# horizon-research/Fov-3DGS

Hardware: AMD Instinct MI355X
Metric: frames/sec at 1080p foveated (bicycle-scale) (higher is better)
Workload: dtype f32; 1 GPU; S-6M bicycle-scale cloud, 4-layer foveated render (fov_pcheck_obb), the reference's 9 fixed gazes (0.25 i, 0.25 j) in turn, one camera per GPU; gaussians=6000000, width=1920, height=1080, sh_degree=3, model_layout=the reference's tensor interface (render(packed=None)), overlap_successive_frames=True, parallelism=views1

## Files before the change

fov-3dgs_amd/csrc/api.hip:

```cpp
#include "common.h"
#include <mutex>
#include <cstdarg>
#include <cstdio>
#include <cstring>
#include <cstdlib>
#include <new>

namespace fr {

static thread_local char g_err[512] = "";

void set_error(const char *fmt, ...)
{
	va_list ap;
	va_start(ap, fmt);
	vsnprintf(g_err, sizeof(g_err), fmt, ap);
	va_end(ap);
}

int check_launch(const char *what, hipStream_t stream, bool debug)
{
	hipError_t e = hipGetLastError();
	static const bool trace = getenv("FR_TRACE") != nullptr;
	if (trace) { fprintf(stderr, "[fovraster] launched %s\n", what); fflush(stderr); }
// ... 189 lines not shown
	c.a = a; c.stream = stream;
	if (a->P == 0)
	{
		FR_HIP(hipMemsetAsync(a->out_color, 0, sizeof(float) * 3 * (size_t)a->W * a->H, stream));
		f->empty = true;
		*out = f; guard.f = nullptr;
		return FR_OK;
	}
	auto mark = [&](int i) { if (a->stage_events && a->stage_events[i]) (void)hipEventRecord((hipEvent_t)a->stage_events[i], stream); };
	c.gx = (a->W + FR_TILE - 1) / FR_TILE; c.gy = (a->H + FR_TILE - 1) / FR_TILE; c.T = c.gx * c.gy;
	c.focal_y = a->H / (2.0f * a->tanfovy);
	c.focal_x = a->W / (2.0f * a->tanfovx);

	char *gptr = a->geometry_resize(a->resize_user[0], carve_geom(a->variant, (size_t)a->P, nullptr).bytes);
	char *iptr = a->image_resize(a->resize_user[2], carve_image(a->variant, a->W, a->H, nullptr).bytes);
	if (!gptr || !iptr) { set_error("geometry/image resize callback returned null"); return FR_ERR_ALLOC; }
	c.geom = carve_geom(a->variant, (size_t)a->P, gptr);
	c.img = carve_image(a->variant, a->W, a->H, iptr);

	c.fov_split = a->variant == FR_VARIANT_FOV_PCHECK_OBB ? 1 : 0;
	f->ax = (!a->debug && !a->no_helper_streams) ? aux_stream(stream) : nullptr;
	hipStream_t fill_stream = stream;
	const bool stats = has_stats(a->variant) && !a->no_stats;
	if (f->ax && (c.fov_split || stats))
	{
		if (hipEventRecord(f->ax->fork, stream) != hipSuccess || hipStreamWaitEvent(f->ax->s2, f->ax->fork, 0) != hipSuccess) { (void)hipGetLastError(); f->ax = nullptr; }
		else fill_stream = f->ax->s2;
	}
	auto fills_done = [&]() { if (fill_stream != stream && hipEventRecord(f->ax->join2, f->ax->s2) == hipSuccess) f->aux_pending = true; };
	if (c.fov_split)
	{
		const hipError_t e = hipMemsetAsync(a->out_color, 0, sizeof(float) * 3 * (size_t)a->W * a->H, fill_stream);
		fills_done();
		if (e != hipSuccess) { set_error("hipMemsetAsync(out_color): %s", hipGetErrorString(e)); return FR_ERR_HIP; }
	}
	if (stats)
	{
		const hipError_t e1 = hipMemsetAsync(a->gaussians_count, 0, sizeof(int32_t) * (size_t)a->P, fill_stream);
		const hipError_t e2 = hipMemsetAsync(a->contributions, 0, sizeof(float) * (size_t)a->P, fill_stream);
		fills_done();
		if (e1 != hipSuccess || e2 != hipSuccess) { set_error("hipMemsetAsync(statistics): %s", hipGetErrorString(e1 != hipSuccess ? e1 : e2)); return FR_ERR_HIP; }
	}
	FR_HIP(hipMemsetAsync(c.img.tile_count, 0, (size_t)((char *)(c.img.lv_bbox + 5 * FR_LV_BBOX_STRIDE) - (char *)c.img.tile_count), stream));
	if (!is_fov(a->variant))
		FR_HIP(hipMemsetAsync(c.geom.slab_ctr, 0, FR_SLAB_CTR_WORDS * sizeof(uint32_t), stream));
	if (a->list_consumed) FR_HIP(hipMemsetAsync(a->list_consumed, 0, sizeof(uint32_t) * (size_t)c.T, stream));
	if (a->blend_pairs) FR_HIP(hipMemsetAsync(a->blend_pairs, 0, sizeof(uint32_t) * (size_t)c.T, stream));
	static thread_local uint32_t frame_seq = 0;
	if (++frame_seq == 0) frame_seq = 1;
	c.totals_seq = frame_seq;
	mark(FR_STAGE_TILE_LEVELS);
	if (is_fov(a->variant)) { rc = launch_tile_levels(c); if (rc) return rc; }
	mark(FR_STAGE_PROJECT);
	rc = launch_project(c); if (rc) return rc;
	int cur_dev = 0;
	(void)hipGetDevice(&cur_dev);
	f->pin = a->debug ? nullptr : take_pinned(cur_dev);
	c.totals_host_dev = f->pin ? f->pin->dev : nullptr;
	c.scan_fused = 0;
	mark(FR_STAGE_BIN);
	f->scan_enqueued = true;
	rc = launch_bin(c); if (rc) return rc;
	mark(FR_STAGE_TILE_SCAN);
	if (!c.scan_fused) { rc = launch_tile_scan(c); if (rc) return rc; }
	*out = f; guard.f = nullptr;
	return FR_OK;
}

// ... 43 lines not shown
	a->num_rendered = (int32_t)totals[0];
	a->max_tile_instances = (int32_t)totals[1];
	a->num_candidates = (int32_t)candidates;
	c.heavy4 = (int)totals[2]; c.heavy2 = (int)totals[3];
	c.n_items = (int)totals[5]; c.heavy8 = (int)totals[6];
	const int64_t want = (int64_t)totals[0] + (int64_t)totals[0] / 4 + 65536;
	if (!same_kind) { gs.variant = a->variant; gs.P = a->P; gs.W = a->W; gs.H = a->H; gs.capacity = 0; }
	if (want > gs.capacity) gs.capacity = want;

	const bool fits_early = early_bin && (int64_t)totals[0] <= early_cap;
	const int64_t capacity = fits_early ? early_cap : (int64_t)totals[0];
	char *bptr = fits_early ? early_bin : a->binning_resize(a->resize_user[1], carve_bin(capacity, nullptr, c.T).bytes);
	if (!bptr) { set_error("binning resize callback returned null"); return FR_ERR_ALLOC; }
	c.bin = carve_bin(capacity, bptr, c.T);
	c.capacity = capacity;
	c.items_cap = (int64_t)(c.fov_split ? 4 : 2) * c.T;
	int rc = FR_OK;
	mark(FR_STAGE_EMIT);
	if (a->num_rendered > 0) { rc = launch_emit(c); if (rc) return rc; }
	mark(FR_STAGE_TILE_SORT);
	if (a->num_rendered > 0) { rc = launch_tile_sort(c); if (rc) return rc; }
	mark(FR_STAGE_RENDER);
	f->join_aux();
	rc = launch_render(c);
	mark(FR_NUM_STAGES);
	return rc;
}

int fr_forward_abandon(fr_frame *f)
{
	if (!f) { set_error("null frame"); return FR_ERR_INVALID; }
	delete f;
	return FR_OK;
}

int fr_forward(fr_forward_args *a)
{
	fr_frame *f = nullptr;
	const int rc = fr_forward_begin(a, &f);
	if (rc) return rc;
	return fr_forward_finish(f);
}

int fr_pack_geom(int32_t P, const float *means3D, const float *scales, const float *rotations, const float *opacities,
	int32_t levels, const float *highest_levels, float *packed_geom, void *stream)
{
// ... 106 lines not shown
```

fov-3dgs_amd/csrc/common.h:

```cpp
#pragma once
#include <hip/hip_runtime.h>
#include <stdint.h>
#include <stddef.h>
#include "../../include/fovraster.h"

#define FR_TILE 16
#define FR_TILE_PIX 256
#define FR_FOV_LEVELS 4
#define FR_SORT_LDS_MAX 8192
#ifndef FR_BIN_THREADS
#define FR_BIN_THREADS 768
#endif
#define FR_BIN_BLOCKS 512
#define FR_PROJ_MAX_WAVES 8192
#define FR_CROW_PAD (64 * FR_PROJ_MAX_WAVES)
#define FR_LDS_HIST_MAX_TILES 16384
#define FR_ITEM_NONE 0xffffffffu
#define FR_LDS_HIST16_MAX_TILES 34816
#define FR_HIST16_MAX_SLABS (65535 / FR_BIN_THREADS)
#define FR_BIG_TNUM 64
#define FR_GIANT_TNUM 1024
#define FR_GIANT_MAX 64
#define FR_SORT_SPLIT_MIN 16384
#define FR_SORT_CHUNK_TARGET 960
#define FR_SORT_FINE_BUCKETS 2048
#define FR_SORT_MAX_CHUNKS(D) ((size_t)(D) / FR_SORT_CHUNK_TARGET + (size_t)(D) / FR_SORT_SPLIT_MIN + 16)
#define FR_LV_BBOX_STRIDE 32
#define FR_SLAB_CTR_WORDS 32

namespace fr {

#define FR_VARIANT_SUM_NOSTATS 100
__host__ __device__ inline bool has_stats(int v) { return v == FR_VARIANT_PCHECK_OBB_SUM || v == FR_VARIANT_PCHECK_OBB_MAX || v == FR_VARIANT_PCHECK_OBB_LWMC; }
__host__ __device__ inline bool has_backward(int v) { return v == FR_VARIANT_ORIGINAL || has_stats(v); }
__host__ __device__ constexpr inline bool is_fov(int v) { return v == FR_VARIANT_FOV_PCHECK_OBB || v == FR_VARIANT_NAIVE_FOV_PCHECK_OBB || v == FR_VARIANT_MMFR_PCHECK_OBB; }

__host__ __device__ inline size_t align_up(size_t x, size_t a = 256) { return (x + a - 1) / a * a; }

struct GeomWS {
	float4 *rec;
	float *cov3D;
	float4 *acc;
	float4 *wrec;
	float4 *lvl;
	uint32_t *lrange;
	uint32_t *slab_ctr;
	uint32_t *vis_list;
	uint32_t *vis_seg;
	uint32_t *proj_counts;
	uint32_t *wbase;
// ... 20 lines not shown
	if (variant == FR_VARIANT_FOV_PCHECK_OBB) { g.lvl = (float4 *)(base + off); off = align_up(off + P * FR_FOV_LEVELS * sizeof(float4)); }
	g.lrange = (uint32_t *)(base + off); off = align_up(off + P * sizeof(uint32_t));
	g.slab_ctr = (uint32_t *)(base + off); off = align_up(off + FR_SLAB_CTR_WORDS * sizeof(uint32_t));
	g.vis_list = (uint32_t *)(base + off); off = align_up(off + P * sizeof(uint32_t));
	g.vis_seg = (uint32_t *)(base + off); off = align_up(off + (P + FR_CROW_PAD) * sizeof(uint32_t));
	g.proj_counts = (uint32_t *)(base + off); off = align_up(off + FR_PROJ_MAX_WAVES * sizeof(uint32_t));
	g.wbase = (uint32_t *)(base + off); off = align_up(off + (FR_PROJ_MAX_WAVES + 1) * sizeof(uint32_t));
	g.crow = nullptr;
	if (is_fov(variant)) { g.crow = (float4 *)(base + off); off = align_up(off + (P + FR_CROW_PAD) * 3 * sizeof(float4)); }
	g.rtab = (uint2 *)(base + off); off = align_up(off + (size_t)FR_BIN_BLOCKS * FR_MAX_REGIONS * sizeof(uint2));
	g.wlist = (uint32_t *)(base + off); off = align_up(off + wlist_cap(P) * sizeof(uint32_t));
	g.rtotal = (uint32_t *)(base + off); off = align_up(off + FR_MAX_REGIONS * sizeof(uint32_t));
	g.rchunk = (uint32_t *)(base + off); off = align_up(off + (FR_MAX_REGIONS + 1) * sizeof(uint32_t));
	g.bytes = off + 256;
	return g;
}

struct ImageWS {
	float *final_T;
	uint32_t *n_contrib;
	uint2 *ranges;
	uint32_t *tile_count;
	uint32_t *lv_bbox;
	uint32_t *totals;
	uint32_t *render_items;
	uint32_t *tile_order;
	float *tile_lv;
	uint32_t *hist;
	size_t bytes;
};
__host__ __device__ inline int bin_blocks(int P)
{
	const int slabs = (P + FR_BIN_THREADS - 1) / FR_BIN_THREADS;
	return slabs < FR_BIN_BLOCKS ? (slabs > 0 ? slabs : 1) : FR_BIN_BLOCKS;
}
__host__ __device__ inline ImageWS carve_image(int variant, int W, int H, char *base)
{
	ImageWS s; size_t off = 0;
	const size_t N = (size_t)W * H;
	const size_t T = (size_t)((W + FR_TILE - 1) / FR_TILE) * ((H + FR_TILE - 1) / FR_TILE);
	s.final_T = (float *)(base + off); off = align_up(off + N * sizeof(float));
	s.n_contrib = (uint32_t *)(base + off); off = align_up(off + N * sizeof(uint32_t));
	s.ranges = (uint2 *)(base + off); off = align_up(off + T * sizeof(uint2));
	s.tile_count = (uint32_t *)(base + off); off = align_up(off + T * sizeof(uint32_t));
	s.lv_bbox = (uint32_t *)(base + off); off = align_up(off + 5 * FR_LV_BBOX_STRIDE * sizeof(uint32_t));
	s.totals = (uint32_t *)(base + off); off = align_up(off + 16 * sizeof(uint32_t));
	s.render_items = (uint32_t *)(base + off); off = align_up(off + 4 * T * sizeof(uint32_t));
	s.tile_order = (uint32_t *)(base + off); off = align_up(off + T * sizeof(uint32_t));
	s.tile_lv = nullptr;
	if (is_fov(variant)) { s.tile_lv = (float *)(base + off); off = align_up(off + 5 * T * sizeof(float)); }
	s.hist = nullptr;
	if (T <= FR_LDS_HIST16_MAX_TILES) { s.hist = (uint32_t *)(base + off); off = align_up(off + (size_t)FR_BIN_BLOCKS * T * sizeof(uint32_t)); }
	s.bytes = off + 256;
	return s;
}

struct BinWS {
	uint32_t *point_list;
	uint64_t *entries;
	uint64_t *entries2;
	uint2 *chunks;
	uint32_t *round_flags;
	size_t bytes;
};
__host__ __device__ inline size_t round_flag_words(int64_t D, int64_t T) { return (size_t)((D / 256 + T + 64) / 32 + 1); }
__host__ __device__ inline BinWS carve_bin(int64_t D, char *base, int64_t T = 1 << 20)
{
	BinWS b; size_t off = 0;
	b.point_list = (uint32_t *)(base + off); off = align_up(off + (size_t)D * sizeof(uint32_t));
	b.entries = (uint64_t *)(base + off); off = align_up(off + (size_t)D * sizeof(uint64_t));
	b.entries2 = (uint64_t *)(base + off); off = align_up(off + (size_t)D * sizeof(uint64_t));
	b.chunks = (uint2 *)(base + off); off = align_up(off + FR_SORT_MAX_CHUNKS(D) * sizeof(uint2));
	b.round_flags = (uint32_t *)(base + off); off = align_up(off + round_flag_words(D, T) * sizeof(uint32_t));
// ... 244 lines not shown
```

fov-3dgs_amd/csrc/preprocess.hip:

```cpp
#include "common.h"
#include "tile_scan.h"
#include <cstdlib>

namespace fr {

struct M3 { float c[3][3]; };
__device__ __forceinline__ M3 m3_cols(float a0, float a1, float a2, float b0, float b1, float b2, float c0, float c1, float c2)
{
	M3 m; m.c[0][0] = a0; m.c[0][1] = a1; m.c[0][2] = a2; m.c[1][0] = b0; m.c[1][1] = b1; m.c[1][2] = b2;
	m.c[2][0] = c0; m.c[2][1] = c1; m.c[2][2] = c2; return m;
}
__device__ __forceinline__ M3 m3_mul(const M3 &a, const M3 &b)
{
	M3 r;
#pragma unroll
	for (int col = 0; col < 3; col++)
#pragma unroll
		for (int row = 0; row < 3; row++)
			r.c[col][row] = a.c[0][row] * b.c[col][0] + a.c[1][row] * b.c[col][1] + a.c[2][row] * b.c[col][2];
	return r;
}
__device__ __forceinline__ M3 m3_t(const M3 &a)
{
	M3 r;
// ... 19 lines not shown
	const float nx = px / W, ny = py / H;
	float tdir[3], gdir[3], cdir[3];
	ncd2dir(nx, ny, riw, rih, tdir);
	ncd2dir(gaze_x, gaze_y, riw, rih, gdir);
	ncd2dir(0.5f, 0.5f, riw, rih, cdir);
	const float ecc = acosf(gdir[0] * tdir[0] + gdir[1] * tdir[1] + gdir[2] * tdir[2]);
	const float ecc_c = acosf(tdir[0] * cdir[0] + tdir[1] * cdir[1] + tdir[2] * cdir[2]);
	const float pool = alpha * ecc * ecc;
	const float amin = (float)((double)ecc_c - (double)pool * 0.5);
	const float amax = (float)((double)ecc_c + (double)pool * 0.5);
	const float ax = (float)(((double)nx - 0.5) * (double)riw), ay = (float)(((double)ny - 0.5) * (double)rih);
	const float dist = sqrtf(ax * ax + ay * ay + rvd * rvd);
	const float major = (tanf(amax) - tanf(amin)) * rvd;
	const float minor = 2.0f * dist * tanf(pool * 0.5f);
	const float area = (float)(3.14159265358979323846 * (double)major * (double)minor * (double)0.25f);
	const float r2p = W / riw;
	const float ps = sqrtf(area) * r2p;
	float level;
	if (ps <= 1) level = 0; else level = (sqrtf(ps) - 1) / step;
	if ((double)level > ((double)(float)FR_FOV_LEVELS - 0.1)) level = (float)((double)(float)FR_FOV_LEVELS - 0.1);
	return level;
}

#define FR_LV_PATCH 14
__global__ void __launch_bounds__(256) k_tile_levels(int T, int gx, int gy, int W, int H, float gaze_x, float gaze_y, float alpha, float *out,
	uint32_t *lv_bbox, uint32_t *slab_ctr, float mmfr_level)
{
	if (blockIdx.x == 0)
		for (int i = threadIdx.x; i < FR_SLAB_CTR_WORDS; i += 256) slab_ctr[i] = 0;
	__shared__ float s_lv[16][16];
	const int pxn = (gx + FR_LV_PATCH - 1) / FR_LV_PATCH;
	const int bx = (int)blockIdx.x % pxn, by = (int)blockIdx.x / pxn;
	const int lx = threadIdx.x & 15, ly = threadIdx.x >> 4;
	const int tx = bx * FR_LV_PATCH + lx - 1, ty = by * FR_LV_PATCH + ly - 1;
	const bool in_grid = tx >= 0 && tx < gx && ty >= 0 && ty < gy;
	const bool live = in_grid && lx >= 1 && lx <= FR_LV_PATCH && ly >= 1 && ly <= FR_LV_PATCH;
	const int idx = ty * gx + tx;
	s_lv[ly][lx] = in_grid ? tile_level(tx, ty, W, H, gaze_x, gaze_y, alpha) : -1.0f;
	__syncthreads();
	const float lf = s_lv[ly][lx];
	const int xl = max(lx - 1, 0), xr = min(lx + 1, 15), yd = max(ly - 1, 0), yu = min(ly + 1, 15);
	const float right = s_lv[ly][xr], left = s_lv[ly][xl], up = s_lv[yu][lx], down = s_lv[yd][lx];
	float gxv = 0, gyv = 0;
	if (right != -1 && left != -1) gxv = (right - left) / 2.0f;
	else if (right != -1) gxv = right - lf;
	else if (left != -1) gxv = lf - left;
	if (up != -1 && down != -1) gyv = (up - down) / 2.0f;
	else if (up != -1) gyv = up - lf;
	else if (down != -1) gyv = lf - down;
	const float max_delta = (float)(0.5 * (double)(fabsf(gxv) + fabsf(gyv)));
	const bool mmfr = mmfr_level >= 0.0f;
	float tmin = lf - max_delta;
	if (mmfr && tmin < 0.0f) tmin = 0.0f;
	const float tmin_i = (float)f2i(tmin);
	const bool blending = ((tmin - tmin_i) > 0.5f) && (tmin_i < (float)(FR_FOV_LEVELS - 1));
	const float real_tmin = tmin;
	if (mmfr) tmin = (real_tmin > mmfr_level - 0.5f && real_tmin < mmfr_level + 1.0f) ? 0.0f : 5.0f;
	if (live)
	{
		out[idx] = mmfr ? real_tmin : lf;
		out[T + idx] = tmin;
		out[2 * T + idx] = gxv;
		out[3 * T + idx] = gyv;
		out[4 * T + idx] = blending ? 1.0f : 0.0f;
	}
	__shared__ uint32_t s_bb[(FR_FOV_LEVELS + 1) * 4];
	if (threadIdx.x < (FR_FOV_LEVELS + 1) * 4) s_bb[threadIdx.x] = 0;
	__syncthreads();
	for (int k = 0; k <= FR_FOV_LEVELS; k++)
	{
		const bool in = live && tmin < (float)k;
		uint32_t v[4] = { in ? (uint32_t)(gx - tx) : 0u, in ? (uint32_t)(gy - ty) : 0u, in ? (uint32_t)(tx + 1) : 0u, in ? (uint32_t)(ty + 1) : 0u };
#pragma unroll
		for (int c = 0; c < 4; c++)
		{
#pragma unroll
			for (int off = 32; off > 0; off >>= 1) v[c] = max(v[c], (uint32_t)__shfl_xor((int)v[c], off));
			if ((threadIdx.x & 63) == 0 && v[c] != 0) atomicMax(&s_bb[4 * k + c], v[c]);
		}
	}
	__syncthreads();
	if (threadIdx.x < (FR_FOV_LEVELS + 1) * 4 && s_bb[threadIdx.x] != 0)
		atomicMax(&lv_bbox[(threadIdx.x >> 2) * FR_LV_BBOX_STRIDE + (threadIdx.x & 3)], s_bb[threadIdx.x]);
}

typedef float f4u __attribute__((ext_vector_type(4), aligned(4)));
struct ShRows { f4u v[12]; };
template <bool REST>
__device__ __forceinline__ void sh_fetch(const float *__restrict__ sh, ShRows &r)
{
#pragma unroll
	for (int q = 0; q < 11; q++) r.v[q] = *(const f4u *)(sh + 4 * q);
	if (REST) r.v[11] = (f4u){ sh[44], 0.0f, 0.0f, 0.0f };
	else r.v[11] = *(const f4u *)(sh + 44);
}
__device__ __forceinline__ void sh_basis(float dx, float dy, float dz, float basis[16])
{
	const float len = sqrtf(dx * dx + dy * dy + dz * dz);
	const float x = dx / len, y = dy / len, z = dz / len;
	const float xx = x * x, yy = y * y, zz = z * z;
	const float xy = x * y, yz = y * z, xz = x * z;
	const float b[16] = {
		FR_SH_C0, -(FR_SH_C1 * y), FR_SH_C1 * z, -(FR_SH_C1 * x),
		FR_SH_C2_0 * xy, FR_SH_C2_1 * yz, FR_SH_C2_2 * (2.0f * zz - xx - yy), FR_SH_C2_3 * xz, FR_SH_C2_4 * (xx - yy),
		FR_SH_C3_0 * y * (3.0f * xx - yy), FR_SH_C3_1 * xy * z, FR_SH_C3_2 * y * (4.0f * zz - xx - yy),
		FR_SH_C3_3 * z * (2.0f * zz - 3.0f * xx - 3.0f * yy), FR_SH_C3_4 * x * (4.0f * zz - xx - yy),
// ... 62 lines not shown
	}
#pragma unroll
	for (int ch = 0; ch < 3; ch++) out[ch] = acc[ch] + 0.5f;
}

typedef float nt_f4 __attribute__((ext_vector_type(4)));
__device__ __forceinline__ float4 nt_load4(const float *p)
{
	const nt_f4 v = __builtin_nontemporal_load((const nt_f4 *)p);
	return make_float4(v.x, v.y, v.z, v.w);
}
struct RawGaussian { float p[3], sc[3]; float4 q; float hl; };

#define FR_ER_CHUNK 512
struct PreArgs {
	int P, D, M, W, H, gx, gy;
	float tanfovx, tanfovy, focal_x, focal_y, scale_modifier;
	const float *means3D, *scales, *rotations, *opacities, *shs, *cov3D_precomp, *colors_precomp;
	const float *shs_rest;
	const float *viewmatrix, *projmatrix, *campos;
	const float *shs_dcs, *highest_levels;
	const float *packed_geom, *packed_colour, *packed_cull;
	const float *tile_lv;
	const uint32_t *lv_bbox;
	int lds_tiles;
	int T;
	int *radii;
	GeomWS geom;
	uint32_t *tile_count;
	uint32_t *hist;
	int write_cov3D;
	int raw;
	int prefiltered;
	int proj_waves, proj_cpw;
	int wbase_lds;
	int fuse_scan;
	TileScanArgs ts;
	int regions, region_rx;
	int wcap;
};

struct Proj {
	bool alive;
	float pix_x, pix_y, depth, conic_a, conic_b, conic_c;
	float cov0, cov1, lambda1, lambda2;
	int radius, x0, y0, x1, y1;
	uint32_t tnum;
// ... 212 lines not shown
{
	if (b <= a) return 0ull;
	const unsigned long long hi = b >= 64 ? ~0ull : ((1ull << b) - 1ull);
	return hi & ~((1ull << a) - 1ull);
}

#ifndef FR_PROJ_THREADS
#define FR_PROJ_THREADS 1024
#endif
#ifndef FR_PROJ_DEPTH
#define FR_PROJ_DEPTH 3
#endif
#ifndef FR_PROJ_DEPTH_PACKED
#define FR_PROJ_DEPTH_PACKED 4
#endif
__host__ __device__ inline int proj_chunks_per_wave(int P, int nwaves) { const int nchunks = (P + 63) / 64; return (nchunks + nwaves - 1) / nwaves; }
template <int VARIANT, bool PACKED = false>
__global__ void __launch_bounds__(FR_PROJ_THREADS) k_project(const PreArgs a)
{
	constexpr int DEPTH = PACKED ? FR_PROJ_DEPTH_PACKED : FR_PROJ_DEPTH;
	constexpr bool FOV = VARIANT == FR_VARIANT_FOV_PCHECK_OBB;
	const int lane = threadIdx.x & 63;
	__shared__ uint4 s_lvb[5];
	if (FOV && threadIdx.x < 5) s_lvb[threadIdx.x] = *(const uint4 *)(a.lv_bbox + threadIdx.x * FR_LV_BBOX_STRIDE);
	if (FOV) __syncthreads();
	constexpr bool ROWS = !PACKED && FOV;
	const int nwaves = (int)gridDim.x * (FR_PROJ_THREADS / 64);
	const int nchunks = (a.P + 63) / 64;
	const int wave_gid = (int)blockIdx.x * (FR_PROJ_THREADS / 64) + (int)(threadIdx.x >> 6);
	const int cpw = proj_chunks_per_wave(a.P, nwaves);
	const int c0 = wave_gid * cpw, c1 = min(nchunks, c0 + cpw);
	const uint32_t row_base = (uint32_t)wave_gid * (uint32_t)cpw * 64u;
	uint32_t nrow = 0;
	const bool have_sr = a.cov3D_precomp == nullptr;
	const float wn2 = view_norm2_bound(a.viewmatrix);
	float vm[16], pm[16];
#pragma unroll
	for (int i = 0; i < 16; i++)
	{
		vm[i] = __builtin_bit_cast(float, __builtin_amdgcn_readfirstlane(__builtin_bit_cast(int, a.viewmatrix[i])));
		pm[i] = __builtin_bit_cast(float, __builtin_amdgcn_readfirstlane(__builtin_bit_cast(int, a.projmatrix[i])));
	}
	const float *sc_src = have_sr ? a.scales : a.cov3D_precomp;
	const float *q_src = have_sr ? a.rotations : a.cov3D_precomp;
	bool odd_level = false;
	auto fetch = [&](const int chunk) __attribute__((always_inline))
	{
		const size_t i = (size_t)min(chunk * 64 + lane, a.P - 1);
// ... 762 lines not shown
				if (t == 0) a.geom.rchunk[a.regions] = tot;
			}
		}
	}
}
#undef BUMP_TILE
#undef TILE_FILTER

struct EmitArgs {
	int P, gx, gy, T;
	const int *radii;
	GeomWS geom;
	const float *highest_levels;
	const float *tile_lv;
	const uint32_t *lv_bbox;
	int lds_tiles;
	const uint2 *ranges;
	uint32_t *cursor;
	uint64_t *entries;
	const uint32_t *hist;
	const uint32_t *totals;
	uint32_t capacity;
	uint32_t items_cap;
};
#ifndef FR_EMIT_THREADS
#define FR_EMIT_THREADS FR_BIN_THREADS
#endif
#ifdef FR_EMIT_NOSTORE
#define FR_EMIT_ST(slot, v) do { if ((slot) == 0xffffffffu) a.entries[0] = (v); } while (0)
#elif defined(FR_EMIT_COALESCED)
#define FR_EMIT_ST(slot, v) do { (void)(slot); a.entries[(size_t)blockIdx.x * 20000 + (threadIdx.x & ~63u) * 26u + ((uint32_t)tm_seq++ * 64u + lane) % 1600u] = (v); } while (0)
#else
#define FR_EMIT_ST(slot, v) a.entries[(slot)] = (v)
#endif
#define NEXT_SLOT(ti) (LDSH == 2 ? a.ranges[(ti)].x + pre_row[(ti)] + ((atomicAdd(&lds_cur[(ti) >> 1], 1u << (16 * ((ti) & 1))) >> (16 * ((ti) & 1))) & 0xffffu) \
	: LDSH ? atomicAdd(&lds_cur[(ti)], 1u) : a.ranges[(ti)].x + atomicAdd(&a.cursor[(ti)], 1u))
template <int VARIANT, int LDSH>
__global__ void __launch_bounds__(FR_EMIT_THREADS) k_emit(const EmitArgs a)
{
	constexpr bool CULL = VARIANT != FR_VARIANT_ORIGINAL;
	constexpr bool FOV = VARIANT == FR_VARIANT_FOV_PCHECK_OBB;
	extern __shared__ __attribute__((aligned(16))) uint32_t lds_cur[];
#ifdef FR_EMIT_TIMERS
	const uint64_t tm_entry = wall_clock64(); uint64_t tm_pro = 0, tm_loop = 0, tm_walk = 0, tm_big = 0, tm_drain = 0, tm_pre = 0, tm_mid = 0, tm_ta = 0; int tm_slabs = 0, tm_steps = 0;
#endif
	if (a.totals[0] > a.capacity || a.totals[5] > a.items_cap) return;
	const int lane = threadIdx.x & 63;
#ifdef FR_EMIT_COALESCED
	uint32_t tm_seq = 0;
#endif
	const int cur_words = LDSH == 2 ? (a.T + 1) / 2 : (LDSH ? a.T : 0);
	const uint32_t *const pre_row = a.hist + (LDSH ? (size_t)blockIdx.x * a.T : 0);
	uint32_t *lds_tab = lds_cur + cur_words;
	const int tab_words = (a.T + 7) / 8;
	const bool ldst = FOV && a.lds_tiles && a.geom.slab_ctr[3] == 0u;
	if (ldst)
	{
		const float *gmin = a.tile_lv + a.T;
		for (int t0 = threadIdx.x; t0 < a.T; t0 += 16 * FR_EMIT_THREADS)
		{
			float v[16];
#pragma unroll
			for (int k = 0; k < 16; k++) v[k] = gmin[min(t0 + k * FR_EMIT_THREADS, a.T - 1)];
#pragma unroll
			for (int k = 0; k < 16; k++)
			{
				const int t = t0 + k * FR_EMIT_THREADS;
				uint32_t nib = t < a.T ? (v[k] == v[k] ? (uint32_t)min(max(f2i(v[k]), 0), 7) : 7u) : 0u;
				nib <<= 4 * (lane & 7);
				nib |= (uint32_t)__shfl_xor((int)nib, 1); nib |= (uint32_t)__shfl_xor((int)nib, 2); nib |= (uint32_t)__shfl_xor((int)nib, 4);
// ... 230 lines not shown
	for (int g = 0; g < ng; g++)
	{
		const float4 *wr = a.geom.wrec + 4 * (size_t)s_gidx[g];
		const float4 w0 = wr[0], w1 = wr[1], w2 = wr[2], w3 = wr[3];
		const Obb ob = make_obb(w0.x, w0.y, make_float4(w0.z, w0.w, w1.x, w1.y), make_float2(w1.z, w1.w));
		const uint32_t xy = __float_as_uint(w2.z);
		const uint64_t opay = ((uint64_t)__float_as_uint(w2.y) << 32) | (uint32_t)s_gidx[g];
		walk_uniform((int)(xy & 0xffffu), (int)(xy >> 16), (int)__float_as_uint(w2.w), __float_as_uint(w3.x), ob, w3.y + 1, opay,
			(uint32_t)(threadIdx.x & ~63u), (uint32_t)FR_EMIT_THREADS);
	}
}
#undef NEXT_SLOT
#undef TILE_PASSES

struct EmitRegArgs {
	int gx, gy, T, RX, R, bin_wgs, wcap;
	GeomWS geom;
	const float *tile_lv;
	const uint2 *ranges;
	uint32_t *cursor;
	uint64_t *entries;
	const uint32_t *totals;
	uint32_t capacity, items_cap;
};
#define FR_ER_THREADS 256
#define FR_ER_WAVES (FR_ER_THREADS / 64)
#define FR_ER_STAGE 384
template <int VARIANT>
__global__ void __launch_bounds__(FR_ER_THREADS) k_emit_regions(const EmitRegArgs a)
{
	constexpr bool CULL = VARIANT != FR_VARIANT_ORIGINAL;
	constexpr bool FOV = VARIANT == FR_VARIANT_FOV_PCHECK_OBB;
	constexpr int RT = FR_REGION_TILES;
	if (a.totals[0] > a.capacity || a.totals[5] > a.items_cap) return;
	__shared__ uint32_t s_rchunk[FR_MAX_REGIONS + 1];
	__shared__ uint32_t s_pre[FR_BIN_BLOCKS + 1], s_src[FR_BIN_BLOCKS], s_part[FR_ER_WAVES], s_chunk;
	__shared__ float s_tmin[RT * RT];
	__shared__ __attribute__((aligned(16))) float4 s_orec[FR_ER_WAVES][64 * 4];
	__shared__ int s_own[FR_ER_WAVES][64];
	__shared__ __attribute__((aligned(8))) uint64_t s_pay[FR_ER_WAVES][FR_ER_STAGE];
	__shared__ uint8_t s_tl[FR_ER_WAVES][FR_ER_STAGE];
	__shared__ uint32_t s_cnt[FR_ER_WAVES][RT * RT], s_base[FR_ER_WAVES][RT * RT];
	const int lane = threadIdx.x & 63, wv = threadIdx.x >> 6;
	for (int t = threadIdx.x; t <= a.R; t += FR_ER_THREADS) s_rchunk[t] = a.geom.rchunk[t];
	__syncthreads();
	const uint32_t nchunks = s_rchunk[a.R];
	float4 *const orec = s_orec[wv];
	uint64_t *const pay = s_pay[wv];
	uint8_t *const stl = s_tl[wv];
	int cur_r = -1, tx0 = 0, ty0 = 0, n = 0, npre = 1;
	uint32_t n_staged = 0;
#ifdef FR_ER_TIMERS
	const uint64_t tm_start = wall_clock64(); uint64_t tm_pro = 0, tm_fetch = 0, tm_proc = 0, tm_flush = 0; int tm_chunks = 0, tm_flushes = 0, tm_regions = 0;
#define ERT(x) x
#else
#define ERT(x)
#endif
// ... 236 lines not shown
	const float *highest_levels, float *out, hipStream_t stream)
{
	const size_t n = (size_t)P * 4;
	hipLaunchKernelGGL(k_pack_geom, dim3((unsigned)((n + 255) / 256)), dim3(256), 0, stream, P, means3D, scales, rotations, opacities, levels,
		highest_levels, (float4 *)out);
	return check_launch("pack_geom", stream, 0);
}
int launch_pack_cull(int P, const float *means3D, const float *scales, const float *rotations, float *out, hipStream_t stream)
{
	hipLaunchKernelGGL(k_pack_cull, dim3((unsigned)(((size_t)P + 255) / 256)), dim3(256), 0, stream, P, means3D, scales, rotations, (float4 *)out);
	return check_launch("pack_cull", stream, 0);
}
int launch_pack_colour(int P, const float *shs, const float *shs_rest, const float *shs_dcs, float *out, hipStream_t stream)
{
	const size_t n = (size_t)P * 64;
	hipLaunchKernelGGL(k_pack_colour, dim3((unsigned)((n + 255) / 256)), dim3(256), 0, stream, P, shs, shs_rest, shs_dcs, out);
	return check_launch("pack_colour", stream, 0);
}

static inline size_t lds_tile_table_bytes(int T) { return (size_t)((T + 7) / 8) * sizeof(uint32_t); }
int launch_tile_levels(FwdCtx &c)
{
	const fr_forward_args *a = c.a;
	hipLaunchKernelGGL(k_tile_levels, dim3(((c.gx + FR_LV_PATCH - 1) / FR_LV_PATCH) * ((c.gy + FR_LV_PATCH - 1) / FR_LV_PATCH)), dim3(256), 0, c.stream,
		c.T, c.gx, c.gy, a->W, a->H, a->gaze_x, a->gaze_y, a->alpha, c.img.tile_lv, c.img.lv_bbox, c.geom.slab_ctr,
		a->variant == FR_VARIANT_MMFR_PCHECK_OBB ? a->cur_level : -1.0f);
	return check_launch("tile_levels", c.stream, a->debug);
}

static PreArgs make_pre_args(FwdCtx &c)
{
	const fr_forward_args *a = c.a;
	PreArgs p;
	p.lds_tiles = 0; p.wbase_lds = 0;
	p.P = a->P; p.D = a->D; p.M = a->M; p.W = a->W; p.H = a->H; p.gx = c.gx; p.gy = c.gy;
	p.tanfovx = a->tanfovx; p.tanfovy = a->tanfovy; p.focal_x = c.focal_x; p.focal_y = c.focal_y;
	p.scale_modifier = a->scale_modifier;
	p.means3D = a->means3D; p.scales = a->scales; p.rotations = a->rotations; p.opacities = a->opacities;
	p.shs = a->shs; p.shs_rest = a->shs_rest; p.cov3D_precomp = a->cov3D_precomp; p.colors_precomp = a->colors_precomp;
	p.viewmatrix = a->viewmatrix; p.projmatrix = a->projmatrix; p.campos = a->campos;
	p.packed_geom = a->packed_geom; p.packed_colour = a->packed_colour; p.packed_cull = a->packed_cull;
	p.shs_dcs = a->shs_dcs; p.highest_levels = a->highest_levels; p.tile_lv = c.img.tile_lv; p.lv_bbox = c.img.lv_bbox; p.T = c.T;
	p.radii = a->radii; p.geom = c.geom; p.tile_count = c.img.tile_count; p.hist = c.img.hist; p.raw = a->raw_activations;
	p.write_cov3D = has_backward(a->variant) ? 1 : 0;
	p.prefiltered = a->prefiltered;
	p.proj_waves = c.proj_waves; p.proj_cpw = c.proj_cpw;
	p.fuse_scan = 0;
	p.regions = 0; p.region_rx = 0; p.wcap = 0;
	return p;
}

int launch_project(FwdCtx &c)
{
	const fr_forward_args *a = c.a;
	PreArgs p = make_pre_args(c);
	{
		static thread_local int resident_of[8][6];
		int cur_dev = 0;
		(void)hipGetDevice(&cur_dev);
		int *const resident = resident_of[cur_dev & 7];
		const bool packed = a->packed_cull != nullptr;
		const int vslot = a->variant == FR_VARIANT_ORIGINAL ? 0 : (is_fov(a->variant) ? 1 : 2);
		const int slot = vslot + (packed ? 3 : 0);
		if (resident[slot] == 0)
		{
// ... 100 lines not shown
	{
	case FR_VARIANT_ORIGINAL: LAUNCH_BIN(FR_VARIANT_ORIGINAL); break;
	case FR_VARIANT_FOV_PCHECK_OBB: LAUNCH_BIN(FR_VARIANT_FOV_PCHECK_OBB); break;
	case FR_VARIANT_MMFR_PCHECK_OBB:
	case FR_VARIANT_NAIVE_FOV_PCHECK_OBB:
		if (crow) LAUNCH_BIN_PC(FR_VARIANT_NAIVE_FOV_PCHECK_OBB, false, true); else LAUNCH_BIN_PC(FR_VARIANT_NAIVE_FOV_PCHECK_OBB, false, false);
		break;
	default: LAUNCH_BIN(FR_VARIANT_PCHECK_OBB); break;
	}
#undef LAUNCH_BIN
#undef LAUNCH_BIN_PC
	if (lrc) return lrc;
	c.bin_wgs = nblk;
	return check_launch("bin", c.stream, a->debug);
}

static int launch_emit_regions(FwdCtx &c)
{
	const fr_forward_args *a = c.a;
	EmitRegArgs e;
	e.gx = c.gx; e.gy = c.gy; e.T = c.T; e.RX = c.region_rx; e.R = c.regions; e.bin_wgs = c.bin_wgs; e.wcap = c.wcap;
	e.geom = c.geom; e.tile_lv = c.img.tile_lv; e.ranges = c.img.ranges; e.cursor = c.img.tile_count; e.entries = c.bin.entries;
	e.totals = c.img.totals; e.capacity = (uint32_t)c.capacity; e.items_cap = (uint32_t)c.items_cap;
	static thread_local int wgs = 0;
	if (wgs == 0)
	{
		int per_cu = 0, dev = 0; hipDeviceProp_t prop;
		if (hipGetDevice(&dev) != hipSuccess || hipGetDeviceProperties(&prop, dev) != hipSuccess ||
			hipOccupancyMaxActiveBlocksPerMultiprocessor(&per_cu, (const void *)k_emit_regions<FR_VARIANT_FOV_PCHECK_OBB>, FR_ER_THREADS, 0) != hipSuccess || per_cu < 1)
		{ per_cu = 4; prop.multiProcessorCount = 256; (void)hipGetLastError(); }
		wgs = per_cu * prop.multiProcessorCount;
	}
	const dim3 grid((unsigned)wgs), block(FR_ER_THREADS);
	switch (a->variant)
	{
	case FR_VARIANT_ORIGINAL: hipLaunchKernelGGL((k_emit_regions<FR_VARIANT_ORIGINAL>), grid, block, 0, c.stream, e); break;
	case FR_VARIANT_FOV_PCHECK_OBB:
	case FR_VARIANT_MMFR_PCHECK_OBB:
	case FR_VARIANT_NAIVE_FOV_PCHECK_OBB: hipLaunchKernelGGL((k_emit_regions<FR_VARIANT_FOV_PCHECK_OBB>), grid, block, 0, c.stream, e); break;
	default: hipLaunchKernelGGL((k_emit_regions<FR_VARIANT_PCHECK_OBB>), grid, block, 0, c.stream, e); break;
	}
	return check_launch("emit_regions", c.stream, a->debug);
}

int launch_emit(FwdCtx &c)
{
	const fr_forward_args *a = c.a;
	if (c.regions && c.regions_ok) return launch_emit_regions(c);
	EmitArgs e;
	e.P = a->P; e.gx = c.gx; e.gy = c.gy; e.T = c.T; e.radii = a->radii; e.geom = c.geom;
	e.highest_levels = a->highest_levels; e.tile_lv = c.img.tile_lv; e.lv_bbox = c.img.lv_bbox; e.ranges = c.img.ranges;
	e.cursor = c.img.tile_count; e.entries = c.bin.entries; e.hist = c.img.hist;
	e.totals = c.img.totals; e.capacity = (uint32_t)c.capacity; e.items_cap = (uint32_t)c.items_cap;
	const bool ldsh = c.hist_mode != 0;
	const dim3 grid(c.bin_wgs), block(FR_EMIT_THREADS);
	e.lds_tiles = (is_fov(a->variant) && ldsh) ? 1 : 0;
	const size_t lds = (((c.hist_mode == 2 ? (size_t)((c.T + 1) / 2) * sizeof(uint32_t) : (ldsh ? (size_t)c.T * sizeof(uint32_t) : 0)) +
		(e.lds_tiles ? lds_tile_table_bytes(c.T) : 0) + 15) & ~(size_t)15) + (size_t)FR_EMIT_THREADS * 4 * sizeof(float4);
	if (lds > 64u * 1024u)
	{
		static const hipError_t once = []() {
			const void *fns[] = { (const void *)k_emit<FR_VARIANT_ORIGINAL, 0>, (const void *)k_emit<FR_VARIANT_ORIGINAL, 1>, (const void *)k_emit<FR_VARIANT_ORIGINAL, 2>,
				(const void *)k_emit<FR_VARIANT_PCHECK_OBB, 0>, (const void *)k_emit<FR_VARIANT_PCHECK_OBB, 1>, (const void *)k_emit<FR_VARIANT_PCHECK_OBB, 2>,
				(const void *)k_emit<FR_VARIANT_FOV_PCHECK_OBB, 0>, (const void *)k_emit<FR_VARIANT_FOV_PCHECK_OBB, 1>, (const void *)k_emit<FR_VARIANT_FOV_PCHECK_OBB, 2> };
			for (const void *fn : fns)
			{
				const hipError_t e1 = hipFuncSetAttribute(fn, hipFuncAttributeMaxDynamicSharedMemorySize, (FR_EMIT_THREADS > 768 ? 154 : 156) * 1024);
				if (e1 != hipSuccess) return e1;
			}
			return hipSuccess; }();
		if (once != hipSuccess) { set_error("hipFuncSetAttribute(k_emit): %s", hipGetErrorString(once)); return FR_ERR_HIP; }
	}
#define LAUNCH_EMIT(V) do { if (c.hist_mode == 2) hipLaunchKernelGGL((k_emit<V, 2>), grid, block, lds, c.stream, e); \
	else if (ldsh) hipLaunchKernelGGL((k_emit<V, 1>), grid, block, lds, c.stream, e); \
	else hipLaunchKernelGGL((k_emit<V, 0>), grid, block, lds, c.stream, e); } while (0)
	switch (a->variant)
// ... 19 lines not shown
```

Measured before the change: 2146 frames/s.

## Drop full-frame memsets; clear only two-level tiles and fold resets into kernels

Removes the full out_color memset on the foveated path. The emit kernels now zero only the pixels of tiles whose render item marks them as two-level (blend) tiles, presumably because the render kernel writes every other pixel itself. The tile_count/lv_bbox memset is also dropped: k_tile_levels zeroes tile_count and writes per-block level-bbox partials instead of using atomicMax. The project kernel then reduces those partials in every block and writes the final bbox. This saves two memset launches and a 25MB clear, at the cost of a redundant reduction in every project block and correctness that depends on render fully covering the remaining tiles.

```diff
diff --git a/fov-3dgs_amd/csrc/api.hip b/fov-3dgs_amd/csrc/api.hip
--- a/fov-3dgs_amd/csrc/api.hip
+++ b/fov-3dgs_amd/csrc/api.hip
@@ -235,18 +235,12 @@
 	f->ax = (!a->debug && !a->no_helper_streams) ? aux_stream(stream) : nullptr;
 	hipStream_t fill_stream = stream;
 	const bool stats = has_stats(a->variant) && !a->no_stats;
-	if (f->ax && (c.fov_split || stats))
+	if (f->ax && stats)
 	{
 		if (hipEventRecord(f->ax->fork, stream) != hipSuccess || hipStreamWaitEvent(f->ax->s2, f->ax->fork, 0) != hipSuccess) { (void)hipGetLastError(); f->ax = nullptr; }
 		else fill_stream = f->ax->s2;
 	}
 	auto fills_done = [&]() { if (fill_stream != stream && hipEventRecord(f->ax->join2, f->ax->s2) == hipSuccess) f->aux_pending = true; };
-	if (c.fov_split)
-	{
-		const hipError_t e = hipMemsetAsync(a->out_color, 0, sizeof(float) * 3 * (size_t)a->W * a->H, fill_stream);
-		fills_done();
-		if (e != hipSuccess) { set_error("hipMemsetAsync(out_color): %s", hipGetErrorString(e)); return FR_ERR_HIP; }
-	}
 	if (stats)
 	{
 		const hipError_t e1 = hipMemsetAsync(a->gaussians_count, 0, sizeof(int32_t) * (size_t)a->P, fill_stream);
@@ -254,9 +248,11 @@
 		fills_done();
 		if (e1 != hipSuccess || e2 != hipSuccess) { set_error("hipMemsetAsync(statistics): %s", hipGetErrorString(e1 != hipSuccess ? e1 : e2)); return FR_ERR_HIP; }
 	}
-	FR_HIP(hipMemsetAsync(c.img.tile_count, 0, (size_t)((char *)(c.img.lv_bbox + 5 * FR_LV_BBOX_STRIDE) - (char *)c.img.tile_count), stream));
 	if (!is_fov(a->variant))
+	{
+		FR_HIP(hipMemsetAsync(c.img.tile_count, 0, (size_t)((char *)(c.img.lv_bbox + 5 * FR_LV_BBOX_STRIDE) - (char *)c.img.tile_count), stream));
 		FR_HIP(hipMemsetAsync(c.geom.slab_ctr, 0, FR_SLAB_CTR_WORDS * sizeof(uint32_t), stream));
+	}
 	if (a->list_consumed) FR_HIP(hipMemsetAsync(a->list_consumed, 0, sizeof(uint32_t) * (size_t)c.T, stream));
 	if (a->blend_pairs) FR_HIP(hipMemsetAsync(a->blend_pairs, 0, sizeof(uint32_t) * (size_t)c.T, stream));
 	static thread_local uint32_t frame_seq = 0;
@@ -346,6 +342,7 @@
 	if (a->num_rendered > 0) { rc = launch_tile_sort(c); if (rc) return rc; }
 	mark(FR_STAGE_RENDER);
 	f->join_aux();
+	if (c.fov_split && a->num_rendered == 0) FR_HIP(hipMemsetAsync(a->out_color, 0, sizeof(float) * 3 * (size_t)a->W * a->H, stream));
 	rc = launch_render(c);
 	mark(FR_NUM_STAGES);
 	return rc;
diff --git a/fov-3dgs_amd/csrc/common.h b/fov-3dgs_amd/csrc/common.h
--- a/fov-3dgs_amd/csrc/common.h
+++ b/fov-3dgs_amd/csrc/common.h
@@ -26,6 +26,8 @@
 #define FR_SORT_FINE_BUCKETS 2048
 #define FR_SORT_MAX_CHUNKS(D) ((size_t)(D) / FR_SORT_CHUNK_TARGET + (size_t)(D) / FR_SORT_SPLIT_MIN + 16)
 #define FR_LV_BBOX_STRIDE 32
+#define FR_LV_PATCH 14
+#define FR_LV_PART_WORDS 32
 #define FR_SLAB_CTR_WORDS 32
 
 namespace fr {
@@ -92,6 +94,7 @@
 	uint2 *ranges;
 	uint32_t *tile_count;
 	uint32_t *lv_bbox;
+	uint32_t *lv_part;
 	uint32_t *totals;
 	uint32_t *render_items;
 	uint32_t *tile_order;
@@ -104,6 +107,7 @@
 	const int slabs = (P + FR_BIN_THREADS - 1) / FR_BIN_THREADS;
 	return slabs < FR_BIN_BLOCKS ? (slabs > 0 ? slabs : 1) : FR_BIN_BLOCKS;
 }
+__host__ __device__ inline int lv_patches(int gx, int gy) { return ((gx + FR_LV_PATCH - 1) / FR_LV_PATCH) * ((gy + FR_LV_PATCH - 1) / FR_LV_PATCH); }
 __host__ __device__ inline ImageWS carve_image(int variant, int W, int H, char *base)
 {
 	ImageWS s; size_t off = 0;
@@ -118,7 +122,13 @@
 	s.render_items = (uint32_t *)(base + off); off = align_up(off + 4 * T * sizeof(uint32_t));
 	s.tile_order = (uint32_t *)(base + off); off = align_up(off + T * sizeof(uint32_t));
 	s.tile_lv = nullptr;
-	if (is_fov(variant)) { s.tile_lv = (float *)(base + off); off = align_up(off + 5 * T * sizeof(float)); }
+	s.lv_part = nullptr;
+	if (is_fov(variant))
+	{
+		s.tile_lv = (float *)(base + off); off = align_up(off + 5 * T * sizeof(float));
+		const int gx = (W + FR_TILE - 1) / FR_TILE, gy = (H + FR_TILE - 1) / FR_TILE;
+		s.lv_part = (uint32_t *)(base + off); off = align_up(off + (size_t)lv_patches(gx, gy) * FR_LV_PART_WORDS * sizeof(uint32_t));
+	}
 	s.hist = nullptr;
 	if (T <= FR_LDS_HIST16_MAX_TILES) { s.hist = (uint32_t *)(base + off); off = align_up(off + (size_t)FR_BIN_BLOCKS * T * sizeof(uint32_t)); }
 	s.bytes = off + 256;
diff --git a/fov-3dgs_amd/csrc/preprocess.hip b/fov-3dgs_amd/csrc/preprocess.hip
--- a/fov-3dgs_amd/csrc/preprocess.hip
+++ b/fov-3dgs_amd/csrc/preprocess.hip
@@ -65,9 +65,8 @@
 	return level;
 }
 
-#define FR_LV_PATCH 14
 __global__ void __launch_bounds__(256) k_tile_levels(int T, int gx, int gy, int W, int H, float gaze_x, float gaze_y, float alpha, float *out,
-	uint32_t *lv_bbox, uint32_t *slab_ctr, float mmfr_level)
+	uint32_t *lv_part, uint32_t *tile_count, uint32_t *slab_ctr, float mmfr_level)
 {
 	if (blockIdx.x == 0)
 		for (int i = threadIdx.x; i < FR_SLAB_CTR_WORDS; i += 256) slab_ctr[i] = 0;
@@ -106,6 +105,7 @@
 		out[2 * T + idx] = gxv;
 		out[3 * T + idx] = gyv;
 		out[4 * T + idx] = blending ? 1.0f : 0.0f;
+		tile_count[idx] = 0;
 	}
 	__shared__ uint32_t s_bb[(FR_FOV_LEVELS + 1) * 4];
 	if (threadIdx.x < (FR_FOV_LEVELS + 1) * 4) s_bb[threadIdx.x] = 0;
@@ -123,8 +123,7 @@
 		}
 	}
 	__syncthreads();
-	if (threadIdx.x < (FR_FOV_LEVELS + 1) * 4 && s_bb[threadIdx.x] != 0)
-		atomicMax(&lv_bbox[(threadIdx.x >> 2) * FR_LV_BBOX_STRIDE + (threadIdx.x & 3)], s_bb[threadIdx.x]);
+	if (threadIdx.x < (FR_FOV_LEVELS + 1) * 4) lv_part[(size_t)blockIdx.x * FR_LV_PART_WORDS + threadIdx.x] = s_bb[threadIdx.x];
 }
 
 typedef float f4u __attribute__((ext_vector_type(4), aligned(4)));
@@ -233,7 +232,9 @@
 	const float *shs_dcs, *highest_levels;
 	const float *packed_geom, *packed_colour, *packed_cull;
 	const float *tile_lv;
-	const uint32_t *lv_bbox;
+	uint32_t *lv_bbox;
+	const uint32_t *lv_part;
+	int lv_parts;
 	int lds_tiles;
 	int T;
 	int *radii;
@@ -492,8 +493,30 @@
 	constexpr bool FOV = VARIANT == FR_VARIANT_FOV_PCHECK_OBB;
 	const int lane = threadIdx.x & 63;
 	__shared__ uint4 s_lvb[5];
-	if (FOV && threadIdx.x < 5) s_lvb[threadIdx.x] = *(const uint4 *)(a.lv_bbox + threadIdx.x * FR_LV_BBOX_STRIDE);
-	if (FOV) __syncthreads();
+	if (FOV)
+	{
+		__shared__ uint32_t s_lvw[(FR_FOV_LEVELS + 1) * 4];
+		static_assert((FR_FOV_LEVELS + 1) * 4 <= 32 && FR_LV_PART_WORDS == 32, "a half-wave per row of lv_part");
+		if (threadIdx.x < (FR_FOV_LEVELS + 1) * 4) s_lvw[threadIdx.x] = 0;
+		const int j = (int)(threadIdx.x & 31);
+		uint32_t m = 0;
+		if (j < (FR_FOV_LEVELS + 1) * 4)
+		{
+#pragma unroll 4
+			for (int w = (int)(threadIdx.x >> 5); w < a.lv_parts; w += FR_PROJ_THREADS / 32) m = max(m, a.lv_part[(size_t)w * FR_LV_PART_WORDS + j]);
+		}
+		m = max(m, (uint32_t)__shfl_xor((int)m, 32));
+		__syncthreads();
+		if (lane < (FR_FOV_LEVELS + 1) * 4 && m != 0) atomicMax(&s_lvw[lane], m);
+		__syncthreads();
+		if (threadIdx.x < 5)
+		{
+			const uint4 b = make_uint4(s_lvw[4 * threadIdx.x], s_lvw[4 * threadIdx.x + 1], s_lvw[4 * threadIdx.x + 2], s_lvw[4 * threadIdx.x + 3]);
+			s_lvb[threadIdx.x] = b;
+			if (blockIdx.x == 0) *(uint4 *)(a.lv_bbox + threadIdx.x * FR_LV_BBOX_STRIDE) = b;
+		}
+		__syncthreads();
+	}
 	constexpr bool ROWS = !PACKED && FOV;
 	const int nwaves = (int)gridDim.x * (FR_PROJ_THREADS / 64);
 	const int nchunks = (a.P + 63) / 64;
@@ -1302,7 +1325,31 @@
 	const uint32_t *totals;
 	uint32_t capacity;
 	uint32_t items_cap;
+	float *out_color;
+	const uint32_t *render_items;
+	int W, H;
 };
+__device__ __forceinline__ void clear_two_level_tiles(float *__restrict__ out_color, const uint32_t *__restrict__ render_items, const uint32_t n_items,
+	const int gx, const int W, const int H, const int wave, const int nwaves, const int lane)
+{
+	const size_t plane = (size_t)W * H;
+	for (uint32_t i0 = (uint32_t)wave * 64u; i0 < n_items; i0 += (uint32_t)nwaves * 64u)
+	{
+		const uint32_t it = i0 + (uint32_t)lane < n_items ? render_items[i0 + lane] : 0u;
+		for (unsigned long long m = __ballot((it & 7u) == 4u); m; m &= m - 1)
+		{
+			const int tile = (int)((uint32_t)__builtin_amdgcn_readlane((int)it, __ffsll((long long)m) - 1) >> 3);
+			const int px = (tile % gx) * FR_TILE + (lane & 15), py0 = (tile / gx) * FR_TILE;
+#pragma unroll
+			for (int k = 0; k < 3 * FR_TILE * FR_TILE / 64; k++)
+			{
+				const int r = k * 4 + (lane >> 4);
+				const int py = py0 + r % FR_TILE;
+				if (px < W && py < H) out_color[(size_t)(r / FR_TILE) * plane + (size_t)W * py + px] = 0.0f;
+			}
+		}
+	}
+}
 #ifndef FR_EMIT_THREADS
 #define FR_EMIT_THREADS FR_BIN_THREADS
 #endif
@@ -1326,6 +1373,9 @@
 #endif
 	if (a.totals[0] > a.capacity || a.totals[5] > a.items_cap) return;
 	const int lane = threadIdx.x & 63;
+	if (FOV && a.out_color)
+		clear_two_level_tiles(a.out_color, a.render_items, a.totals[5], a.gx, a.W, a.H, (int)blockIdx.x * (FR_EMIT_THREADS / 64) + (int)(threadIdx.x >> 6),
+			(int)gridDim.x * (FR_EMIT_THREADS / 64), lane);
 #ifdef FR_EMIT_COALESCED
 	uint32_t tm_seq = 0;
 #endif
@@ -1602,6 +1652,9 @@
 	uint64_t *entries;
 	const uint32_t *totals;
 	uint32_t capacity, items_cap;
+	float *out_color;
+	const uint32_t *render_items;
+	int W, H;
 };
 #define FR_ER_THREADS 256
 #define FR_ER_WAVES (FR_ER_THREADS / 64)
@@ -1613,6 +1666,9 @@
 	constexpr bool FOV = VARIANT == FR_VARIANT_FOV_PCHECK_OBB;
 	constexpr int RT = FR_REGION_TILES;
 	if (a.totals[0] > a.capacity || a.totals[5] > a.items_cap) return;
+	if (FOV && a.out_color)
+		clear_two_level_tiles(a.out_color, a.render_items, a.totals[5], a.gx, a.W, a.H, (int)blockIdx.x * FR_ER_WAVES + (int)(threadIdx.x >> 6),
+			(int)gridDim.x * FR_ER_WAVES, (int)(threadIdx.x & 63));
 	__shared__ uint32_t s_rchunk[FR_MAX_REGIONS + 1];
 	__shared__ uint32_t s_pre[FR_BIN_BLOCKS + 1], s_src[FR_BIN_BLOCKS], s_part[FR_ER_WAVES], s_chunk;
 	__shared__ float s_tmin[RT * RT];
@@ -1895,8 +1951,8 @@
 int launch_tile_levels(FwdCtx &c)
 {
 	const fr_forward_args *a = c.a;
-	hipLaunchKernelGGL(k_tile_levels, dim3(((c.gx + FR_LV_PATCH - 1) / FR_LV_PATCH) * ((c.gy + FR_LV_PATCH - 1) / FR_LV_PATCH)), dim3(256), 0, c.stream,
-		c.T, c.gx, c.gy, a->W, a->H, a->gaze_x, a->gaze_y, a->alpha, c.img.tile_lv, c.img.lv_bbox, c.geom.slab_ctr,
+	hipLaunchKernelGGL(k_tile_levels, dim3(lv_patches(c.gx, c.gy)), dim3(256), 0, c.stream,
+		c.T, c.gx, c.gy, a->W, a->H, a->gaze_x, a->gaze_y, a->alpha, c.img.tile_lv, c.img.lv_part, c.img.tile_count, c.geom.slab_ctr,
 		a->variant == FR_VARIANT_MMFR_PCHECK_OBB ? a->cur_level : -1.0f);
 	return check_launch("tile_levels", c.stream, a->debug);
 }
@@ -1914,6 +1970,7 @@
 	p.viewmatrix = a->viewmatrix; p.projmatrix = a->projmatrix; p.campos = a->campos;
 	p.packed_geom = a->packed_geom; p.packed_colour = a->packed_colour; p.packed_cull = a->packed_cull;
 	p.shs_dcs = a->shs_dcs; p.highest_levels = a->highest_levels; p.tile_lv = c.img.tile_lv; p.lv_bbox = c.img.lv_bbox; p.T = c.T;
+	p.lv_part = c.img.lv_part; p.lv_parts = is_fov(a->variant) ? lv_patches(c.gx, c.gy) : 0;
 	p.radii = a->radii; p.geom = c.geom; p.tile_count = c.img.tile_count; p.hist = c.img.hist; p.raw = a->raw_activations;
 	p.write_cov3D = has_backward(a->variant) ? 1 : 0;
 	p.prefiltered = a->prefiltered;
@@ -2060,6 +2117,7 @@
 	e.gx = c.gx; e.gy = c.gy; e.T = c.T; e.RX = c.region_rx; e.R = c.regions; e.bin_wgs = c.bin_wgs; e.wcap = c.wcap;
 	e.geom = c.geom; e.tile_lv = c.img.tile_lv; e.ranges = c.img.ranges; e.cursor = c.img.tile_count; e.entries = c.bin.entries;
 	e.totals = c.img.totals; e.capacity = (uint32_t)c.capacity; e.items_cap = (uint32_t)c.items_cap;
+	e.out_color = c.fov_split ? a->out_color : nullptr; e.render_items = c.img.render_items; e.W = a->W; e.H = a->H;
 	static thread_local int wgs = 0;
 	if (wgs == 0)
 	{
@@ -2090,6 +2148,7 @@
 	e.highest_levels = a->highest_levels; e.tile_lv = c.img.tile_lv; e.lv_bbox = c.img.lv_bbox; e.ranges = c.img.ranges;
 	e.cursor = c.img.tile_count; e.entries = c.bin.entries; e.hist = c.img.hist;
 	e.totals = c.img.totals; e.capacity = (uint32_t)c.capacity; e.items_cap = (uint32_t)c.items_cap;
+	e.out_color = c.fov_split ? a->out_color : nullptr; e.render_items = c.img.render_items; e.W = a->W; e.H = a->H;
 	const bool ldsh = c.hist_mode != 0;
 	const dim3 grid(c.bin_wgs), block(FR_EMIT_THREADS);
 	e.lds_tiles = (is_fov(a->variant) && ldsh) ? 1 : 0;
```

Result: faster. 2194 frames/s (median of 6 runs) (+2.2%).
